# atonderski/future-object-detection

Measured on AMD Instinct MI355X. Metric: frame-sequences/sec fwd+bwd, T=6 900x1600, higher is better.
Workload: dtype bf16; 1 GPU; spatiotemporal ConditionalDETR (ResNet-50, 6 enc + 6 dec layers, 128 queries), T=6 frames 900x1600, batch 2/GPU, num_images K=5 (5 past frames live), random-init weights; step = forward (incl. Hungarian set loss, post-proc, AP bookkeeping) + backward + clip + AdamW; global_batch=2, frames=6, num_images=5, parallelism=dp1

## Files before the change

### future-object-detection_amd/csrc/stem_pool.hip

```cpp
#include "common.h"

#ifdef FOD_STAMPS
#define SP_MARK(i)                                                           \
  do {                                                                       \
    if (blockIdx.x == 0 && threadIdx.x == 0) {                               \
      const long long now__ = wall_clock64();                                \
      fod_stamps[i] += now__ - mark__;                                       \
      mark__ = now__;                                                        \
    }                                                                        \
  } while (0)
#else
#define SP_MARK(i) \
  do {             \
  } while (0)
#endif

namespace {

constexpr int TP = 8, TQ = 15;
constexpr int SR = 2 * TP + 1;
constexpr int IR = 2 * SR + 5, IC = 72;
constexpr int ROWB_S = 32 * 128;
constexpr int S_OFF = 0, I_OFF = SR * ROWB_S;
constexpr int SH_OFF = I_OFF + IR * IC * 8;
constexpr int LDS_SP = SH_OFF + 256;
constexpr int NPIECE = IR * (IC / 2);
constexpr int PPT = (NPIECE + 255) / 256;

struct StemPoolParams {
  const __bf16* xp;
  const __bf16* w;
  const float* shift;
  __bf16* y;
  int N, Hp, Wp, Ho, Wo, Po, Qo;
};

FOD_DEVINL int at_s(int px, int c16) { return px * 128 + (((c16 ^ (px >> 1)) & 7) << 4); }

typedef unsigned short u16x2 __attribute__((ext_vector_type(2)));

FOD_DEVINL unsigned pk_max_u16(unsigned a, unsigned b) {
  const u16x2 m = __builtin_elementwise_max(__builtin_bit_cast(u16x2, a), __builtin_bit_cast(u16x2, b));
  return __builtin_bit_cast(unsigned, m);
}
FOD_DEVINL uint4 max_u16x8(uint4 a, uint4 b) {
  return make_uint4(pk_max_u16(a.x, b.x), pk_max_u16(a.y, b.y), pk_max_u16(a.z, b.z), pk_max_u16(a.w, b.w));
}

__global__ __launch_bounds__(256, 1) void stem_pool_kernel(const StemPoolParams p) {
  extern __shared__ __attribute__((aligned(16))) unsigned char smem_sp[];
  const int tid = threadIdx.x, lane = tid & 63;
  const int wave = __builtin_amdgcn_readfirstlane(tid >> 6);
  const int fr = lane & 31, fh = lane >> 5;
  unsigned char* S = smem_sp + S_OFF;
  unsigned char* IW = smem_sp + I_OFF;
  float* sshift = reinterpret_cast<float*>(smem_sp + SH_OFF);
  if (tid < 64) sshift[tid] = p.shift ? p.shift[tid] : 0.f;

  const int tq = (p.Qo + TQ - 1) / TQ, tp = (p.Po + TP - 1) / TP;
  const int ntiles = p.N * tp * tq;
  const int per = (ntiles + (int)gridDim.x - 1) / (int)gridDim.x;
  const int lo = (int)blockIdx.x * per, hi = min(ntiles, lo + per);
  if (lo >= hi) return;

  Frag<__bf16> a[2][14];
#pragma unroll
  for (int ct = 0; ct < 2; ++ct)
#pragma unroll
    for (int ks = 0; ks < 14; ++ks)
      a[ct][ks].v = *reinterpret_cast<const bf16x8_t*>(p.w + (long)(32 * ct + fr) * 224 + 16 * ks + 8 * fh);

  auto tile_coords = [&](int t, int& n, int& py0, int& px0) {
    n = t / (tp * tq);
    const int rem = t - n * tp * tq, ti = rem / tq;
    py0 = ti * TP;
    px0 = (rem - ti * tq) * TQ;
  };
  static_assert(PPT == 6, "six staging registers below");
  uint4 pre0, pre1, pre2, pre3, pre4, pre5;
#define FOD_SP_REQ1(J, V)                                                                                        \
  do {                                                                                                           \
    const int i__ = min(tid + 256 * (J), NPIECE - 1);                                                            \
    const int row__ = i__ / (IC / 2), pc__ = i__ - row__ * (IC / 2);                                             \
                                                                                \
    const int hr__ = min(max(hr0__ + row__, 0), p.Hp - 1), hc__ = min(max(hc0__ + 2 * pc__, 0), p.Wp - 2);       \
    V = *reinterpret_cast<const uint4*>(img__ + ((long)hr__ * p.Wp + hc__) * 4);                                 \
  } while (0)
#define FOD_SP_REQUEST(T_)                                                                                       \
  do {                                                                                                           \
    int n__, py__, px__;                                                                                         \
    tile_coords(min((T_), hi - 1), n__, py__, px__);        \
    const int hr0__ = 2 * (2 * py__ - 1), hc0__ = 2 * (2 * px__ - 1);    \
    const __bf16* img__ = p.xp + (long)n__ * p.Hp * p.Wp * 4;                                                    \
    FOD_SP_REQ1(0, pre0); FOD_SP_REQ1(1, pre1); FOD_SP_REQ1(2, pre2);                                            \
    FOD_SP_REQ1(3, pre3); FOD_SP_REQ1(4, pre4); FOD_SP_REQ1(5, pre5);                                            \
  } while (0)
#define FOD_SP_COM1(J, V)                                                              \
  do {                                                                                 \
    const int i__ = tid + 256 * (J);                                                   \
    if (i__ < NPIECE) *reinterpret_cast<uint4*>(IW + i__ * 16) = V;                    \
  } while (0)
#define FOD_SP_COMMIT()                                                                \
  do {                                                                                 \
    FOD_SP_COM1(0, pre0); FOD_SP_COM1(1, pre1); FOD_SP_COM1(2, pre2);                  \
    FOD_SP_COM1(3, pre3); FOD_SP_COM1(4, pre4); FOD_SP_COM1(5, pre5);                  \
  } while (0)
  FOD_SP_REQUEST(lo);
  FOD_SP_COMMIT();
  __syncthreads();

#ifdef FOD_STAMPS
  long long mark__ = wall_clock64();
#endif
  for (int tile = lo; tile < hi; ++tile) {
    int n, py0, px0;
    tile_coords(tile, n, py0, px0);
    const int ho0 = 2 * py0 - 1, wo0 = 2 * px0 - 1;
    FOD_SP_REQUEST(tile + 1);
    for (int lr = wave; lr < SR; lr += 4) {
      f32x16 acc[2];
#pragma unroll
      for (int ct = 0; ct < 2; ++ct)
#pragma unroll
        for (int q = 0; q < 16; ++q) acc[ct][q] = 0.f;
      const unsigned char* rowp = IW + (2 * lr) * (IC * 8) + fr * 16 + fh * 16;
#pragma unroll
      for (int ks = 0; ks < 14; ++ks) {
        Frag<__bf16> b;
        b.v = *reinterpret_cast<const bf16x8_t*>(rowp + (ks >> 1) * (IC * 8) + (ks & 1) * 32);
        mma16(a[0][ks], b, acc[0]);
        mma16(a[1][ks], b, acc[1]);
      }
      const int ho = ho0 + lr, wo = wo0 + fr;
      const bool inside = ho >= 0 && ho < p.Ho && wo >= 0 && wo < p.Wo;
#pragma unroll
      for (int ct = 0; ct < 2; ++ct)
#pragma unroll
        for (int g = 0; g < 4; ++g) {
          const f32x4 sh = *reinterpret_cast<const f32x4*>(sshift + 32 * ct + 8 * g + 4 * fh);
          bf16x4_t o;
#pragma unroll
          for (int e = 0; e < 4; ++e) o[e] = (__bf16)(inside ? fmaxf(acc[ct][4 * g + e] + sh[e], 0.f) : 0.f);
          *reinterpret_cast<bf16x4_t*>(S + lr * ROWB_S + at_s(fr, 4 * ct + g) + 8 * fh) = o;
        }
    }
    SP_MARK(0);
    __syncthreads();
    SP_MARK(1);
    FOD_SP_COMMIT();
    for (int it = tid; it < TP * TQ * 8; it += 256) {
      const int c16 = it & 7, pq = it >> 3;
      const int pp = pq / TQ, qq = pq - pp * TQ;
      const int py = py0 + pp, px = px0 + qq;
      uint4 m = *reinterpret_cast<const uint4*>(S + (2 * pp) * ROWB_S + at_s(2 * qq, c16));
#pragma unroll
      for (int d = 1; d < 9; ++d) {
        const int dy = d / 3, dx = d - 3 * dy;
        m = max_u16x8(m, *reinterpret_cast<const uint4*>(S + (2 * pp + dy) * ROWB_S + at_s(2 * qq + dx, c16)));
      }
      if (py < p.Po && px < p.Qo) *reinterpret_cast<uint4*>(p.y + (((long)n * p.Po + py) * p.Qo + px) * 64 + c16 * 8) = m;
    }
    SP_MARK(2);
    __syncthreads();
    SP_MARK(3);
  }
#undef FOD_SP_REQUEST
#undef FOD_SP_COMMIT
#undef FOD_SP_REQ1
#undef FOD_SP_COM1
}

}

extern "C" int fod_stem_pool_fwd(int dtype, const void* xp, const void* w, const float* shift, void* y, int Nimg, int Hp,
                                 int Wp, int Ho, int Wo, int Cout, hipStream_t stream) {
  FOD_REQUIRE(dtype == FOD_BF16, "stem_pool: bf16 only (dtype %d)", dtype);
  FOD_REQUIRE(xp && w && y, "stem_pool: null operand");
  FOD_REQUIRE(Cout == 64, "stem_pool: built for the 64-channel ResNet stem (Cout %d)", Cout);
  FOD_REQUIRE(Nimg > 0 && Ho > 0 && Wo > 0, "stem_pool: bad extents");
  FOD_REQUIRE(Hp >= 2 * Ho + 5 && Wp >= 2 * Wo + 6 && Wp % 2 == 0,
              "stem_pool: haloed image %dx%d too small for %dx%d outputs (need >= %dx%d, even width)", Hp, Wp, Ho, Wo,
              2 * Ho + 5, 2 * Wo + 6);
  FOD_REQUIRE(((uintptr_t)xp % 16) == 0 && ((uintptr_t)w % 16) == 0 && ((uintptr_t)y % 16) == 0,
              "stem_pool: operands must be 16-byte aligned");
  StemPoolParams p{};
  p.xp = (const __bf16*)xp; p.w = (const __bf16*)w; p.shift = shift; p.y = (__bf16*)y;
  p.N = Nimg; p.Hp = Hp; p.Wp = Wp; p.Ho = Ho; p.Wo = Wo;
  p.Po = (Ho - 1) / 2 + 1;
  p.Qo = (Wo - 1) / 2 + 1;
  const long ntiles = (long)Nimg * ceil_div(p.Po, TP) * ceil_div(p.Qo, TQ);
  FOD_REQUIRE(ntiles < (1L << 30), "stem_pool: too many tiles");
  int dev = 0, cus = 256;
  if (hipGetDevice(&dev) != hipSuccess || hipDeviceGetAttribute(&cus, hipDeviceAttributeMultiprocessorCount, dev) != hipSuccess) cus = 256;
  static LdsLimitOnce once;
  if (int rc = fod_lds_limit_once(once, reinterpret_cast<const void*>(&stem_pool_kernel), LDS_SP, "stem_pool")) return rc;
  hipLaunchKernelGGL(stem_pool_kernel, dim3((unsigned)(ntiles < cus ? ntiles : cus)), dim3(256), LDS_SP, stream, p);
  FOD_LAUNCH_CHECK();
  return FOD_OK;
}
```

Before: 108.6 frame-sequences/s.

## Split stem conv work by channel half per wave and software-pipeline fragment loads

Each wave now owns one 32-channel half and every other output row, instead of all 64 channels for every fourth row. This halves the weight fragments each wave keeps in registers and lets B-fragment LDS loads for the next row, and the epilogue of the previous row, interleave with the current row's MFMAs under scheduling barriers. The shift vector is held in registers instead of LDS, and the ReLU plus bounds mask is folded into a single fmed3 clamp. The per-wave row deal is asymmetric, nine rows for two waves and eight for the others, and the fixed schedule depends on static_asserts about the tile sizes.

```diff
diff --git a/future-object-detection_amd/csrc/stem_pool.hip b/future-object-detection_amd/csrc/stem_pool.hip
--- a/future-object-detection_amd/csrc/stem_pool.hip
+++ b/future-object-detection_amd/csrc/stem_pool.hip
@@ -22,8 +22,8 @@
 constexpr int IR = 2 * SR + 5, IC = 72;
 constexpr int ROWB_S = 32 * 128;
 constexpr int S_OFF = 0, I_OFF = SR * ROWB_S;
-constexpr int SH_OFF = I_OFF + IR * IC * 8;
-constexpr int LDS_SP = SH_OFF + 256;
+constexpr int LDS_SP = I_OFF + IR * IC * 8;
+constexpr int NITEM = (2 * SR + 3) / 4;
 constexpr int NPIECE = IR * (IC / 2);
 constexpr int PPT = (NPIECE + 255) / 256;
 
@@ -36,7 +36,6 @@
 };
 
 FOD_DEVINL int at_s(int px, int c16) { return px * 128 + (((c16 ^ (px >> 1)) & 7) << 4); }
-
 typedef unsigned short u16x2 __attribute__((ext_vector_type(2)));
 
 FOD_DEVINL unsigned pk_max_u16(unsigned a, unsigned b) {
@@ -45,6 +44,23 @@
 }
 FOD_DEVINL uint4 max_u16x8(uint4 a, uint4 b) {
   return make_uint4(pk_max_u16(a.x, b.x), pk_max_u16(a.y, b.y), pk_max_u16(a.z, b.z), pk_max_u16(a.w, b.w));
+}
+
+FOD_DEVINL void load_frag(Frag<__bf16>& b, const unsigned char* rowp, int ks) {
+  b.v = *reinterpret_cast<const bf16x8_t*>(rowp + (ks >> 1) * (IC * 8) + (ks & 1) * 32);
+}
+
+FOD_DEVINL void epilogue_slice(int s, float (&t)[4], unsigned char* dst, const f32x16& acc, const f32x4& sh, float lim) {
+  const int g = s / 3, ph = s - 3 * g;
+  if (ph < 2) {
+    t[2 * ph] = __builtin_amdgcn_fmed3f(acc[4 * g + 2 * ph] + sh[2 * ph], 0.f, lim);
+    t[2 * ph + 1] = __builtin_amdgcn_fmed3f(acc[4 * g + 2 * ph + 1] + sh[2 * ph + 1], 0.f, lim);
+  } else {
+    bf16x4_t o;
+#pragma unroll
+    for (int e = 0; e < 4; ++e) o[e] = (__bf16)t[e];
+    *reinterpret_cast<bf16x4_t*>(dst) = o;
+  }
 }
 
 __global__ __launch_bounds__(256, 1) void stem_pool_kernel(const StemPoolParams p) {
@@ -54,8 +70,6 @@
   const int fr = lane & 31, fh = lane >> 5;
   unsigned char* S = smem_sp + S_OFF;
   unsigned char* IW = smem_sp + I_OFF;
-  float* sshift = reinterpret_cast<float*>(smem_sp + SH_OFF);
-  if (tid < 64) sshift[tid] = p.shift ? p.shift[tid] : 0.f;
 
   const int tq = (p.Qo + TQ - 1) / TQ, tp = (p.Po + TP - 1) / TP;
   const int ntiles = p.N * tp * tq;
@@ -63,12 +77,24 @@
   const int lo = (int)blockIdx.x * per, hi = min(ntiles, lo + per);
   if (lo >= hi) return;
 
-  Frag<__bf16> a[2][14];
-#pragma unroll
-  for (int ct = 0; ct < 2; ++ct)
-#pragma unroll
-    for (int ks = 0; ks < 14; ++ks)
-      a[ct][ks].v = *reinterpret_cast<const bf16x8_t*>(p.w + (long)(32 * ct + fr) * 224 + 16 * ks + 8 * fh);
+  const int ct = wave & 1, r0 = wave >> 1;
+  const bool nine = r0 == 0;
+  static_assert(NITEM == 9 && SR == 2 * NITEM - 1, "the deal below: rows r0 + 2 j, j < NITEM - r0");
+
+  Frag<__bf16> a[14];
+#pragma unroll
+  for (int ks = 0; ks < 14; ++ks)
+    a[ks].v = *reinterpret_cast<const bf16x8_t*>(p.w + (long)(32 * ct + fr) * 224 + 16 * ks + 8 * fh);
+  f32x4 sh[4];
+#pragma unroll
+  for (int g = 0; g < 4; ++g) {
+    sh[g] = f32x4{0.f, 0.f, 0.f, 0.f};
+    if (p.shift) sh[g] = *reinterpret_cast<const f32x4*>(p.shift + 32 * ct + 8 * g + 4 * fh);
+  }
+  const unsigned char* rowp0 = IW + (2 * r0) * (IC * 8) + fr * 16 + fh * 16;
+  unsigned char* dst0[4];
+#pragma unroll
+  for (int g = 0; g < 4; ++g) dst0[g] = S + r0 * ROWB_S + at_s(fr, 4 * ct + g) + 8 * fh;
 
   auto tile_coords = [&](int t, int& n, int& py0, int& px0) {
     n = t / (tp * tq);
@@ -117,32 +143,40 @@
     tile_coords(tile, n, py0, px0);
     const int ho0 = 2 * py0 - 1, wo0 = 2 * px0 - 1;
     FOD_SP_REQUEST(tile + 1);
-    for (int lr = wave; lr < SR; lr += 4) {
-      f32x16 acc[2];
-#pragma unroll
-      for (int ct = 0; ct < 2; ++ct)
-#pragma unroll
-        for (int q = 0; q < 16; ++q) acc[ct][q] = 0.f;
-      const unsigned char* rowp = IW + (2 * lr) * (IC * 8) + fr * 16 + fh * 16;
-#pragma unroll
-      for (int ks = 0; ks < 14; ++ks) {
-        Frag<__bf16> b;
-        b.v = *reinterpret_cast<const bf16x8_t*>(rowp + (ks >> 1) * (IC * 8) + (ks & 1) * 32);
-        mma16(a[0][ks], b, acc[0]);
-        mma16(a[1][ks], b, acc[1]);
+    const float collim = (wo0 + fr >= 0 && wo0 + fr < p.Wo) ? __builtin_inff() : 0.f;
+    Frag<__bf16> b[2][14];
+    f32x16 acc[2];
+#pragma unroll
+    for (int ks = 0; ks < 14; ++ks) load_frag(b[0][ks], rowp0, ks);
+    __builtin_amdgcn_sched_barrier(0);
+#pragma unroll
+    for (int j = 0; j <= NITEM; ++j) {
+      const bool run = j < NITEM - 1 || (j == NITEM - 1 && nine);
+      const bool fin = j > 0 && (j < NITEM || nine);
+      const int hp = ho0 + r0 + 2 * (j - 1);
+      const float lim = (hp >= 0 && hp < p.Ho) ? collim : 0.f;
+      if (run) {
+        const unsigned char* nextp = rowp0 + ((j + 1 < NITEM - 1 || nine) ? (j + 1) * (4 * IC * 8) : j * (4 * IC * 8));
+        float t[4];
+#pragma unroll
+        for (int q = 0; q < 16; ++q) acc[j & 1][q] = 0.f;
+#pragma unroll
+        for (int ks = 0; ks < 14; ++ks) {
+          mma16(a[ks], b[j & 1][ks], acc[j & 1]);
+          if (j + 1 < NITEM) {
+            if (ks == 0) load_frag(b[(j + 1) & 1][0], nextp, 0);
+            if (ks < 13) load_frag(b[(j + 1) & 1][ks + 1], nextp, ks + 1);
+          }
+          if (j > 0 && ks >= 1 && ks <= 12)
+            epilogue_slice(ks - 1, t, dst0[(ks - 1) / 3] + (j - 1) * (2 * ROWB_S), acc[(j - 1) & 1], sh[(ks - 1) / 3], lim);
+          __builtin_amdgcn_sched_barrier(0);
+        }
+      } else if (fin) {
+        float t[4];
+#pragma unroll
+        for (int s = 0; s < 12; ++s)
+          epilogue_slice(s, t, dst0[s / 3] + (j - 1) * (2 * ROWB_S), acc[(j - 1) & 1], sh[s / 3], lim);
       }
-      const int ho = ho0 + lr, wo = wo0 + fr;
-      const bool inside = ho >= 0 && ho < p.Ho && wo >= 0 && wo < p.Wo;
-#pragma unroll
-      for (int ct = 0; ct < 2; ++ct)
-#pragma unroll
-        for (int g = 0; g < 4; ++g) {
-          const f32x4 sh = *reinterpret_cast<const f32x4*>(sshift + 32 * ct + 8 * g + 4 * fh);
-          bf16x4_t o;
-#pragma unroll
-          for (int e = 0; e < 4; ++e) o[e] = (__bf16)(inside ? fmaxf(acc[ct][4 * g + e] + sh[e], 0.f) : 0.f);
-          *reinterpret_cast<bf16x4_t*>(S + lr * ROWB_S + at_s(fr, 4 * ct + g) + 8 * fh) = o;
-        }
     }
     SP_MARK(0);
     __syncthreads();
```

Measured after the change: 109.1 frame-sequences/s, median of 6. About the same (+0.5%).
